# hkust-vgd/scanobjectnn

Measured on NVIDIA H100. Metric: point-clouds/sec (B=32, N=2048, 15-class), higher is better.
Workload: dtype f32

## Files before the change

### scanobjectnn_b200/csrc/tc_mlp.cu

```cuda
#include <float.h>
#include <stdlib.h>

#include <atomic>
#include <type_traits>

#include "common.cuh"
#include "mlp_internal.cuh"
#include "ring_gemm.cuh"
#include "tc_common.cuh"

namespace psa {

using namespace tc;

constexpr int kMaxTcLayers = 2;


struct TcArgs {
    long long groups;
    int K;
    int n, m;
    const float* xyz;
    const float* new_xyz;
    const float* uf;
// ... 674 lines not shown
                    }
                }
            } else {
#pragma unroll
                for (int e = 0; e < 2; ++e) {
                    const float m = warp_rowmax16(u.v[0] ? y[0][e] : -FLT_MAX, u.v[1] ? y[1][e] : -FLT_MAX);
                    if (g == 0) sm.red[0][warp][cl + e] = m;
                }
            }
        }
        if (a.pool_k == 1) {
            if (a.stat_partial != nullptr) {
                unit_bar_sync(1, kRingConsumers);
                if (tid < 64) {
                    const int cl = cl0 + tid;
                    float t0 = 0.f, t1 = 0.f;
                    for (int w = 0; w < 8; ++w) { t0 += sm.red[0][w][cl]; t1 += sm.red[1][w][cl]; }
                    float* dst = a.stat_partial + (size_t)u.tile * 2 * a.N;
                    dst[u.col0 + cl] = t0;
                    dst[a.N + u.col0 + cl] = t1;
                }
            }
        } else {
            unit_bar_sync(1, kRingConsumers);
            const bool big = a.pool_k > 128;
            const int wpg = big ? 8 : a.pool_k / 16;
            for (int e = tid; e < (8 / wpg) * 64; e += kRingConsumers) {
                const int grp = e / 64, cl = cl0 + e % 64;
                const long long rs = u.tile * 128 + grp * wpg * 16;
                if (rs >= a.rows) continue;
                float mx = sm.red[0][grp * wpg][cl];
                for (int w = 1; w < wpg; ++w) mx = fmaxf(mx, sm.red[0][grp * wpg + w][cl]);
                const long long wg = rs / a.pool_k;
                if (!big) {
                    a.out[(size_t)wg * a.N + u.col0 + cl] = mx;
                } else {
                    int code = __float_as_int(mx);
                    code = code >= 0 ? code : code ^ 0x7fffffff;
                    atomicMax(reinterpret_cast<int*>(a.out) + (size_t)wg * a.N + u.col0 + cl, code);
                }
            }
        }
    }
};

template <int NP, int NC>
__global__ void __launch_bounds__(kRingThreads, 1) tc_dense_kernel(const __grid_constant__ TcDenseArgs a) {
    ring_gemm<NP, NC>(DenseOp<NP, NC>{a}, a.ring);
}

static_assert(ring_stages(2, 1, DenseOp<2, 1>::kBudget) == 4 && ring_stages(3, 1, DenseOp<3, 1>::kBudget) == 3 &&
              ring_stages(2, 2, DenseOp<2, 2>::kBudget) == 3 && ring_stages(3, 2, DenseOp<3, 2>::kBudget) == 2, "stages of the dense ring");
static const RingKernels kDenseRing = {{{(const void*)tc_dense_kernel<2, 1>, (const void*)tc_dense_kernel<2, 2>},
                                        {(const void*)tc_dense_kernel<3, 1>, (const void*)tc_dense_kernel<3, 2>}},
                                       "tc_dense_kernel", DenseOp<2, 1>::kBudget};

bool tc_dense_eligible(long long rows, int K, int N, int pool_k) {
    if (rows < 128 || K < 32 || N < 64 || (N % 64) != 0) return false;
    if (N > 64 && (N % 128) != 0) return false;
    if (!(pool_k == 1 || pool_k == 32 || pool_k == 64 || (pool_k >= 128 && pool_k % 128 == 0))) return false;
    if (pool_k > 1 && rows % pool_k != 0) return false;
    return true;
}

static std::atomic<int> g_tc_np{2};
int tc_np() { return g_tc_np; }

static size_t tc_dense_image_off3(int K, int N) { return tc_image_alloc_bytes((K + 63) & ~63, N, 2); }
size_t tc_dense_image_bytes(int K, int N) { return tc_dense_image_off3(K, N) + tc_image_alloc_bytes((K + 63) & ~63, N, 3); }

static size_t tc_plan_image_bytes(int Kp, int N) { return g_tc_np == 2 ? tc_image_alloc_bytes(Kp, N, 2) + tc_image_alloc_bytes(Kp, N, 3) : tc_image_alloc_bytes(Kp, N, 3); }

int tc_dense_nt(long long rows, int N) {
    const bool wide = (N % 128) == 0 && 2 * ((rows + 127) / 128 * (N / 128)) > kNumSMs;
    return (wide ? 128 : 64) | image_flag(g_tc_np);
}

int build_image(int K, int Kp, int N, int Nt, const float* W, uint8_t* image, cudaStream_t st, const unsigned int* run_if) {
    if (Nt & kImageF16x2) {
        unsigned int* trailer = reinterpret_cast<unsigned int*>(image + tc_image_trailer_off(Kp, N, 2));
        float* colscale = reinterpret_cast<float*>(image + tc_image_colscale_off(Kp, N, 2));
        PSA_CUDA(cudaMemsetAsync(trailer, 0, 256, st));
        tc_col_scale_kernel<<<(N + 31) / 32, dim3(32, 8), 0, st>>>(K, N, W, colscale, trailer);
        int rc = check_launch("tc_col_scale_kernel");
        if (rc != PSA_OK) return rc;
        tc_prep_weights_kernel<2><<<(Kp * N + 255) / 256, 256, 0, st>>>(K, Kp, N, Nt & ~kImageFlags, W, colscale, image, run_if);
    } else {
        tc_prep_weights_kernel<3><<<(Kp * N + 255) / 256, 256, 0, st>>>(K, Kp, N, Nt & ~kImageFlags, W, nullptr, image, run_if);
    }
    return check_launch("tc_prep_weights_kernel");
}
const unsigned int* image_trailer(const uint8_t* image, int Kp, int N) {
    return reinterpret_cast<const unsigned int*>(image + tc_image_trailer_off(Kp, N, 2));
}
const float* image_colscale(const uint8_t* image, int Kp, int N) {
    return reinterpret_cast<const float*>(image + tc_image_colscale_off(Kp, N, 2));
}

constexpr int kTileCounterWords = PSA_MAX_MLP_LAYERS;

static long long tc_dense_units(long long rows, int N, int Nt) { return (rows + 127) / 128 * (N / Nt); }

int launch_tc_dense(long long rows, int K, int N, int pool_k, int relu, const float* x, const float* W, const float* scale,
                    const float* shift, float* out, const uint8_t* prebuilt, uint8_t* ws_img, unsigned int* flag, unsigned int* counters,
                    cudaStream_t st, const float* xyz3 = nullptr, const float* w3 = nullptr, const float* group_add = nullptr,
                    long long group_rows = 0) {
    const int Kp = (K + 63) & ~63;
    const int Nt = tc_dense_nt(rows, N) & ~kImageFlags;
    TcDenseArgs a;
    a.rows = rows; a.K = K; a.Kp = Kp; a.N = N; a.pool_k = pool_k; a.relu = relu;
    a.x = x; a.scale = scale; a.shift = shift; a.out = out; a.xyz3 = xyz3; a.w3 = w3;
    a.group_add = group_add; a.group_rows = group_rows;
    RingPool pool;
    if (pool_k > 128) { pool.out = out; pool.count = rows / pool_k * N; }
    return ring_run(kDenseRing, a, tc_dense_units(rows, N, Nt), RingWeights{K, Kp, N, Nt, W, ws_img, ws_img + tc_dense_image_off3(K, N), prebuilt},
                    flag, counters, st, pool);
}

bool tc_train_fwd_eligible(long long rows, int K, int N) {
    return rows >= 128 && K >= 128 && K <= 512 && N >= 128 && (N % 128) == 0;
}
int launch_tc_dense_train(long long rows, int K, int N, const float* x, const float* in_scale, const float* in_shift, int in_relu,
                          const float* W, const float* bias, float* y, float* stat_partial, uint8_t* image_ws, cudaStream_t st) {
    const int Kp = (K + 63) & ~63;
    int rc = build_image(K, Kp, N, 128 | kImageBf16x3, W, image_ws, st);
    if (rc != PSA_OK) return rc;
    TcDenseArgs a;
    a.rows = rows; a.K = K; a.Kp = Kp; a.N = N; a.pool_k = 1; a.relu = 0;
    a.x = x; a.scale = nullptr; a.shift = bias; a.out = y; a.xyz3 = nullptr; a.w3 = nullptr;
    a.in_scale = in_scale; a.in_shift = in_shift; a.in_relu = in_relu; a.stat_partial = stat_partial;
    a.ring.image = image_ws;
    return ring_launch(kDenseRing, 3, 128, &a, tc_dense_units(rows, N, 128), st);
}

static const uint8_t* prebuilt_image(const psa_mlp* mlp, int l, int row0, int Nt) {
    if (mlp->image[l] != nullptr && mlp->image_nt[l] == Nt && mlp->image_row0[l] == row0) return reinterpret_cast<const uint8_t*>(mlp->image[l]);
    return nullptr;
}

bool tc_sa_eligible(const psa_mlp* mlp, int c, int nsample, TcArgs* out, int np) {
    if (mlp->n_layers < 2 || mlp->n_layers > 1 + kMaxTcLayers) return false;
    if (!(nsample == 32 || nsample == 64 || nsample == 128)) return false;
    if (mlp->channels[0] != 3 + c) return false;
    const int C1 = mlp->channels[1];
    if (!(C1 == 64 || C1 == 128)) return false;
    TcArgs a{};
    a.C1 = C1;
    a.nl = mlp->n_layers - 1;
    a.np = np;
    for (int l = 0; l < a.nl; ++l) {
        a.Kd[l] = mlp->channels[1 + l];
        a.Ntot[l] = mlp->channels[2 + l];
        if (!(a.Kd[l] == 64 || a.Kd[l] == 128)) return false;
        const bool is_last = (l == a.nl - 1);
        if (!is_last && !(a.Ntot[l] == 64 || a.Ntot[l] == 128)) return false;
        if (is_last && !(a.Ntot[l] == 64 || a.Ntot[l] % 128 == 0)) return false;
    }
    a.stream_last = 0;
    if (tc_sa_layout(a).total + 1024 > kSmemBudget) a.stream_last = 1;
    if (tc_sa_layout(a).total + 1024 > kSmemBudget) return false;
    *out = a;
    return true;
}
bool tc_sa_eligible(const psa_mlp* mlp, int c, int nsample, TcArgs* out) {
    TcArgs a3;
    if (!tc_sa_eligible(mlp, c, nsample, &a3, 3)) return false;
    if (g_tc_np == 3) { *out = a3; return true; }
    return tc_sa_eligible(mlp, c, nsample, out, 2);
}

size_t tc_sa_workspace_bytes(const TcArgs& a, int b, int n, int c) {
    size_t bytes = 256;
    for (int l = 0; l < a.nl; ++l) bytes += tc_image_alloc_bytes(a.Kd[l], a.Ntot[l], 2) + tc_image_alloc_bytes(a.Kd[l], a.Ntot[l], 3);
    if (c > 0) bytes += (((size_t)b * n * a.C1 * sizeof(float) + 255) & ~(size_t)255) + tc_dense_image_bytes(c, a.C1);
    return bytes;
}

static int tc_sa_image_nt() { return kSaNt | image_flag(g_tc_np); }

template <int NP, int C1, int NL, int N0>
static int launch_tc_sa_shape(const TcArgs& a, long long ctas_needed, size_t smem, cudaStream_t st) {
    PSA_CUDA(cudaFuncSetAttribute(tc_sa_kernel<NP, C1, NL, N0>, cudaFuncAttributeMaxDynamicSharedMemorySize, (int)smem));
    int dev = 0, sms = 0, per_sm = 0;
    PSA_CUDA(cudaGetDevice(&dev));
    PSA_CUDA(cudaDeviceGetAttribute(&sms, cudaDevAttrMultiProcessorCount, dev));
    PSA_CUDA(cudaOccupancyMaxActiveBlocksPerMultiprocessor(&per_sm, tc_sa_kernel<NP, C1, NL, N0>, kSaThreads, smem));
    const long long resident = (long long)sms * (per_sm > 0 ? per_sm : 1);
    const int ctas = (int)(ctas_needed < 1 ? 1 : ctas_needed < resident ? ctas_needed : resident);
    tc_sa_kernel<NP, C1, NL, N0><<<ctas, kSaThreads, smem, st>>>(a);
    return check_launch("tc_sa_kernel");
}

template <int NP>
static int launch_tc_sa_np(TcArgs& a, cudaStream_t st) {
    const uint32_t limit = 223u * 1024u;
    a.joint = a.K == 128 || a.stream_last;
    if (!a.joint && tc_sa_layout(a).total + 1024 + sa_carry_bytes(a) + sa_red_bytes(1) > limit) a.joint = 1;
    const size_t used = (size_t)tc_sa_layout(a).total + 1024 + sa_carry_bytes(a);
    const int ncl = a.Ntot[a.nl - 1] / 64;
    a.pool_chunks = 1;
    if (!a.stream_last)
        for (int ng = ncl; ng > 1; --ng)
            if (ncl % ng == 0 && used + sa_red_bytes(ng) <= limit) { a.pool_chunks = ng; break; }
    const int C = sa_chunk(a.K, a.joint);
    const long long nchunks = (a.groups + C - 1) / C;
    const long long ctas_needed = a.joint ? nchunks : (nchunks + 1) / 2;
    const size_t smem = used + sa_red_bytes(a.pool_chunks);
    if (a.nl == 1) return a.C1 == 64 ? launch_tc_sa_shape<NP, 64, 1, 0>(a, ctas_needed, smem, st) : launch_tc_sa_shape<NP, 128, 1, 0>(a, ctas_needed, smem, st);
    if (a.C1 == 64) return a.Ntot[0] == 64 ? launch_tc_sa_shape<NP, 64, 2, 64>(a, ctas_needed, smem, st) : launch_tc_sa_shape<NP, 64, 2, 128>(a, ctas_needed, smem, st);
    return a.Ntot[0] == 64 ? launch_tc_sa_shape<NP, 128, 2, 64>(a, ctas_needed, smem, st) : launch_tc_sa_shape<NP, 128, 2, 128>(a, ctas_needed, smem, st);
}

static int tc_sa_run(TcArgs& a, int b, int n, int m, int c, int nsample, const float* xyz, const float* new_xyz, const float* points,
                     const int* idx, const psa_mlp* mlp, const float* w1c, float* out, void* workspace, cudaStream_t st) {
    int rc = PSA_OK;
    uint8_t* ws = reinterpret_cast<uint8_t*>(workspace);
    unsigned int* words = reinterpret_cast<unsigned int*>(ws);
    PSA_CUDA(cudaMemsetAsync(ws, 0, 256, st));
    ws += 256;
    uint8_t* img2[kMaxTcLayers];
    uint8_t* img3[kMaxTcLayers];
    for (int l = 0; l < a.nl; ++l) {
        img2[l] = ws; ws += tc_image_alloc_bytes(a.Kd[l], a.Ntot[l], 2);
        img3[l] = ws; ws += tc_image_alloc_bytes(a.Kd[l], a.Ntot[l], 3);
    }
    const float* uf = nullptr;
    if (c > 0) {
        float* ufw = reinterpret_cast<float*>(ws);
        uint8_t* uimg = ws + (((size_t)b * n * a.C1 * sizeof(float) + 255) & ~(size_t)255);
        const float* w1f = mlp->weight[0] + (size_t)3 * a.C1;
        if (tc_dense_eligible((long long)b * n, c, a.C1, 1)) {
            rc = launch_tc_dense((long long)b * n, c, a.C1, 1, 0, points, w1f, nullptr, nullptr, ufw, prebuilt_image(mlp, 0, 3, tc_dense_nt((long long)b * n, a.C1)),
                                 uimg, words + 3, words + 4, st);
        } else {
            DenseArgs d;
            d.rows = (long long)b * n; d.K = c; d.N = a.C1; d.pool_k = 1; d.relu = 0;
            d.x = points; d.W = w1f; d.scale = nullptr; d.shift = nullptr; d.out = ufw;
            rc = launch_dense(d, st);
        }
        if (rc != PSA_OK) return rc;
        uf = ufw;
    }
    auto fill = [&](TcArgs& t) {
        t.groups = (long long)b * m; t.K = nsample; t.n = n; t.m = m;
        t.xyz = xyz; t.new_xyz = new_xyz; t.idx = idx; t.out = out; t.uf = uf;
        t.w1x = mlp->weight[0]; t.s1 = mlp->scale[0]; t.t1 = mlp->shift[0]; t.relu1 = mlp->relu[0];
        t.ovf = nullptr; t.run_if = nullptr; t.w1c = w1c;
        for (int l = 0; l < t.nl; ++l) {
            t.s[l] = mlp->scale[1 + l]; t.t[l] = mlp->shift[1 + l]; t.relu[l] = mlp->relu[1 + l]; t.wflag[l] = nullptr; t.colscale[l] = nullptr;
        }
    };
    fill(a);
    for (int l = 0; l < a.nl; ++l) {
        const int nt_img = tc_sa_image_nt();
        const uint8_t* pre = prebuilt_image(mlp, 1 + l, 0, nt_img);
        uint8_t* own = a.np == 2 ? img2[l] : img3[l];
        if (pre == nullptr) { rc = build_image(a.Kd[l], a.Kd[l], a.Ntot[l], nt_img, mlp->weight[1 + l], own, st); if (rc != PSA_OK) return rc; }
        a.image[l] = pre ? pre : own;
        if (a.np == 2) { a.wflag[l] = image_trailer(a.image[l], a.Kd[l], a.Ntot[l]); a.colscale[l] = image_colscale(a.image[l], a.Kd[l], a.Ntot[l]); }
    }
    a.tile_counter = words;
    if (a.np == 3) return launch_tc_sa_np<3>(a, st);
    a.ovf = words + 2;
    rc = launch_tc_sa_np<2>(a, st);
    if (rc != PSA_OK) return rc;
    TcArgs a3;
    PSA_REQUIRE(tc_sa_eligible(mlp, c, nsample, &a3, 3), "sa_module: internal error (bf16x3 eligibility)");
    fill(a3);
    for (int l = 0; l < a3.nl; ++l) {
        const uint8_t* pre = prebuilt_image(mlp, 1 + l, 0, kSaNt | kImageF16x2);
        if (pre != nullptr) {
            a3.image[l] = pre + tc_image_alloc_bytes(a3.Kd[l], a3.Ntot[l], 2);
        } else {
            rc = build_image(a3.Kd[l], a3.Kd[l], a3.Ntot[l], kSaNt | kImageBf16x3, mlp->weight[1 + l], img3[l], st, words + 2);
            if (rc != PSA_OK) return rc;
            a3.image[l] = img3[l];
        }
    }
    a3.tile_counter = words + 1;
    a3.run_if = words + 2;
    return launch_tc_sa_np<3>(a3, st);
}

struct TcGroupAllArgs {
    int c;
    int N[3];
    int Nt[3];
    const float* points;
    const float* xyz;
    const float* w3;
    const uint8_t* image[3];
    const float* colscale[3];
    const unsigned int* wflag[3];
    const float* scale[3];
    const float* shift[3];
    int relu[3];
    float* out;
    unsigned int* ovf;
};

constexpr int kGaStages = 3;
constexpr uint32_t kGaStageBytes = 32768u;
constexpr uint32_t kGaSmemBudget = 222u * 1024u;
__host__ __device__ inline uint32_t group_all_smem(int W0, int W1, int W2) {
    return 1024u + kGaStages * kGaStageBytes + (uint32_t)(W0 + W1) / 64u * kRingXBytes + 12u * (uint32_t)(W0 + W1 + W2);
}

__device__ __forceinline__ uint32_t cluster_ctarank() {
    uint32_t r;
    asm volatile("mov.u32 %0, %%cluster_ctarank;\n" : "=r"(r));
    return r;
}
__device__ __forceinline__ uint32_t mapa_shared(uint32_t addr, uint32_t rank) {
    uint32_t r;
    asm volatile("mapa.shared::cluster.u32 %0, %1, %2;\n" : "=r"(r) : "r"(addr), "r"(rank));
    return r;
}
__device__ __forceinline__ float2 ld_cluster_f32x2(uint32_t addr) {
    float2 v;
    asm volatile("ld.shared::cluster.v2.f32 {%0, %1}, [%2];\n" : "=f"(v.x), "=f"(v.y) : "r"(addr) : "memory");
    return v;
}
__device__ __forceinline__ void cluster_sync_all() {
    asm volatile("barrier.cluster.arrive.release.aligned;\n\tbarrier.cluster.wait.acquire.aligned;\n" ::: "memory");
}
__device__ __forceinline__ void mbar_arrive_cluster(uint32_t addr) {
    asm volatile("fence.acq_rel.cluster;\n\tmbarrier.arrive.release.cluster.shared::cluster.b64 _, [%0];\n" ::"r"(addr) : "memory");
}
__device__ __forceinline__ void mbar_wait_cluster(uint64_t* bar, uint32_t parity) {
    uint32_t done;
    const uint32_t addr = smem_u32(bar);
    do {
        asm volatile(
            "{\n\t.reg .pred p;\n\t"
            "mbarrier.try_wait.parity.acquire.cluster.shared::cta.b64 p, [%1], %2;\n\t"
            "selp.u32 %0, 1, 0, p;\n\t}\n"
            : "=r"(done)
            : "r"(addr), "r"(parity)
            : "memory");
    } while (!done);
}

template <int NC0, int NC1>
__global__ void __cluster_dims__(4, 1, 1) __launch_bounds__(kRingThreads, 1)
tc_group_all_kernel(const __grid_constant__ TcGroupAllArgs a) {
    constexpr int NP = 2, S = kGaStages;
    constexpr uint32_t piece = 8192u, chunk = 16384u;
    extern __shared__ uint8_t smem_raw[];
    __shared__ __align__(8) uint64_t s_full[S], s_empty[S], s_ready[2], s_done;
    __shared__ float s_red[8][128];
    const int tid = threadIdx.x, lane = tid & 31, warp = tid >> 5;
    const uint32_t rank = cluster_ctarank();
    const int cloud = blockIdx.x >> 2;
    uint8_t* base = smem_raw + ((1024u - (smem_u32(smem_raw) & 1023u)) & 1023u);
    constexpr int W0 = 64 * NC0, W1 = 64 * NC1;
    const int W2 = a.N[2] / 4;
    uint8_t* slice0 = base + S * kGaStageBytes;
    uint8_t* slice1 = slice0 + NC0 * kRingXBytes;
    float* aff0 = reinterpret_cast<float*>(slice1 + NC1 * kRingXBytes);
    float* aff1 = aff0 + 3 * W0;
    float* aff2 = aff1 + 3 * W1;
    {
        float* aff[3] = {aff0, aff1, aff2};
        const int W[3] = {W0, W1, W2};
#pragma unroll
        for (int l = 0; l < 3; ++l)
            for (int i = tid; i < W[l]; i += kRingThreads) {
                const int col = (int)rank * W[l] + i;
                const float cs = __ldg(a.colscale[l] + col);
                aff[l][i] = (a.scale[l] ? __ldg(a.scale[l] + col) : 1.f) * cs;
                aff[l][W[l] + i] = a.shift[l] ? __ldg(a.shift[l] + col) : 0.f;
                aff[l][2 * W[l] + i] = pow2_rcp(cs);
            }
    }
    if (tid == 0) {
        for (int i = 0; i < S; ++i) { mbar_init(&s_full[i], 1); mbar_init(&s_empty[i], kRingConsumers / 32); }
        mbar_init(&s_ready[0], 4); mbar_init(&s_ready[1], 4); mbar_init(&s_done, 4);
        fence_mbar_init();
    }
    __syncthreads();
    cluster_sync_all();
    const int KC[3] = {a.c / 64, 4 * W0 / 64, 4 * W1 / 64};

    if (warp >= kRingConsumers / 32) {
        asm volatile("setmaxnreg.dec.sync.aligned.u32 40;\n");
        if (warp != kRingConsumers / 32) return;
        uint32_t u = 0;
#pragma unroll
        for (int l = 0; l < 3; ++l) {
            const int pw = l == 0 ? W0 : l == 1 ? W1 : 128, passes = l == 2 ? W2 / 128 : 1, Nt = a.Nt[l];
            for (int p = 0; p < passes; ++p) {
                const int j0 = ((int)rank * (l == 0 ? W0 : l == 1 ? W1 : W2) + p * pw) / 64;
                for (int kb = 0; kb < KC[l]; ++kb, ++u) {
                    const int s = (int)(u % S);
                    if (u >= (uint32_t)S) mbar_wait(&s_empty[s], ((u / S) - 1u) & 1u);
                    if (lane == 0) {
                        mbar_expect_tx(&s_full[s], (uint32_t)(pw / 64) * chunk);
                        for (int c = 0; c < pw / 64; ++c) {
                            uint8_t* dst = base + (uint32_t)s * kGaStageBytes + (uint32_t)c * chunk;
                            const int j = j0 + c;
                            if (Nt == 64) {
                                bulk_g2s(dst, a.image[l] + ((size_t)j * KC[l] + kb) * chunk, chunk, &s_full[s]);
                            } else {
                                const uint8_t* src = a.image[l] + ((size_t)(j >> 1) * KC[l] + kb) * (2u * chunk) + (uint32_t)(j & 1) * piece;
                                bulk_g2s(dst, src, piece, &s_full[s]);
                                bulk_g2s(dst + piece, src + 2u * piece, piece, &s_full[s]);
                            }
                        }
                    }
                }
            }
        }
        return;
    }

    asm volatile("setmaxnreg.inc.sync.aligned.u32 232;\n");
    const int g = lane >> 2, t = lane & 3;
    const int rl[2] = {warp * 16 + g, warp * 16 + g + 8};
    uint32_t ovf = 0u;
    uint32_t u = 0;

    auto pass = [&](auto Ltag, auto NCtag, int lc) {
        constexpr int L = decltype(Ltag)::value, NC = decltype(NCtag)::value;
        const int nkb = KC[L];
        auto prep = [&](uint32_t (&A)[NP][4][4], int kb) {
            if constexpr (L == 0) {
                const float* xb = a.points + (size_t)cloud * 128 * a.c + kb * 64;
#pragma unroll
                for (int s = 0; s < 4; ++s)
#pragma unroll
                    for (int h = 0; h < 2; ++h)
#pragma unroll
                        for (int i = 0; i < 2; ++i) {
                            const float2 x = __ldg(reinterpret_cast<const float2*>(xb + (size_t)rl[i] * a.c + 16 * s + 8 * h + 2 * t));
                            put_a<NP, 4>(A, s, i + 2 * h, x.x, x.y, ovf);
                        }
            } else {
                constexpr int Wp = L == 1 ? W0 : W1;
                const uint32_t src = mapa_shared(smem_u32(L == 1 ? slice0 : slice1) + (uint32_t)((kb * 64) % Wp / 64) * kRingXBytes,
                                                 (uint32_t)(kb * 64 / Wp));
#pragma unroll
                for (int s = 0; s < 4; ++s)
#pragma unroll
                    for (int h = 0; h < 2; ++h)
#pragma unroll
                        for (int i = 0; i < 2; ++i) {
                            const float2 x = ld_cluster_f32x2(src + (uint32_t)rl[i] * kRingXRow + (uint32_t)(16 * s + 8 * h + 2 * t) * 4u);
                            put_a<NP, 4>(A, s, i + 2 * h, x.x, x.y, ovf);
                        }
            }
        };
        float acc[NC][32];
        auto step = [&](const uint32_t (&A)[NP][4][4], uint32_t (&An)[NP][4][4], int kb) {
            const int s = (int)(u % S);
            mbar_wait(&s_full[s], (u / S) & 1u);
            const uint32_t wb = smem_u32(base) + (uint32_t)s * kGaStageBytes;
            float d[NC][32];
            wg_fence();
#pragma unroll
            for (int tt = 0; tt < Split<NP>::kTerms; ++tt)
#pragma unroll
                for (int ks = 0; ks < 4; ++ks)
#pragma unroll
                    for (int c = 0; c < NC; ++c)
                        wg_mma_rs<NP>(d[c], A[Split<NP>::a(tt)][ks][0], A[Split<NP>::a(tt)][ks][1], A[Split<NP>::a(tt)][ks][2], A[Split<NP>::a(tt)][ks][3],
                                      wg_desc(wb + (uint32_t)c * chunk + Split<NP>::w(tt) * piece + (uint32_t)ks * 32u), (tt | ks) ? 1u : 0u);
            wg_commit();
            if (kb + 1 < nkb) prep(An, kb + 1);
            wg_wait_all();
            __syncwarp();
            if (lane == 0) mbar_arrive1(&s_empty[s]);
            ++u;
#pragma unroll
            for (int c = 0; c < NC; ++c) {
                wg_fence_acc(d[c]);
#pragma unroll
                for (int e = 0; e < 32; ++e) acc[c][e] = kb ? acc[c][e] + d[c][e] : d[c][e];
            }
        };
        {
            uint32_t A0[NP][4][4], A1[NP][4][4];
            prep(A0, 0);
            for (int kb = 0;; kb += 2) {
                step(A0, A1, kb);
                if (kb + 1 == nkb) break;
                step(A1, A0, kb + 1);
                if (kb + 2 == nkb) break;
            }
        }

        constexpr int W = L == 0 ? W0 : L == 1 ? W1 : 0;
        const int Wl = L == 2 ? W2 : W;
        const float* aff = L == 0 ? aff0 : L == 1 ? aff1 : aff2;
        float xs[2][3] = {{0.f, 0.f, 0.f}, {0.f, 0.f, 0.f}};
        if constexpr (L == 0)
#pragma unroll
            for (int i = 0; i < 2; ++i)
#pragma unroll
                for (int k = 0; k < 3; ++k) xs[i][k] = __ldg(a.xyz + ((size_t)cloud * 128 + rl[i]) * 3 + k);
#pragma unroll
        for (int c = 0; c < NC; ++c)
#pragma unroll
            for (int j = 0; j < 8; ++j) {
                const int cl = c * 64 + 8 * j + 2 * t, ls = lc + cl;
                float y[2][2];
#pragma unroll
                for (int e = 0; e < 2; ++e) {
                    const float sc = aff[ls + e], sh = aff[Wl + ls + e];
                    float w0 = 0.f, w1 = 0.f, w2 = 0.f;
                    if constexpr (L == 0) {
                        const int col = (int)rank * W0 + ls + e;
                        const float f = aff[2 * Wl + ls + e];
                        w0 = __ldg(a.w3 + col) * f; w1 = __ldg(a.w3 + a.N[0] + col) * f; w2 = __ldg(a.w3 + 2 * a.N[0] + col) * f;
                    }
#pragma unroll
                    for (int i = 0; i < 2; ++i) {
                        float x = acc[c][4 * j + 2 * i + e];
                        if constexpr (L == 0) x = fmaf(xs[i][2], w2, fmaf(xs[i][1], w1, fmaf(xs[i][0], w0, x)));
                        x = fmaf(x, sc, sh);
                        if (a.relu[L]) x = fmaxf(x, 0.f);
                        y[i][e] = x;
                    }
                }
                if constexpr (L < 2) {
                    uint8_t* sl = (L == 0 ? slice0 : slice1) + (ls >> 6) * kRingXBytes + (ls & 63) * 4;
#pragma unroll
                    for (int i = 0; i < 2; ++i) *reinterpret_cast<float2*>(sl + rl[i] * kRingXRow) = make_float2(y[i][0], y[i][1]);
                } else {
#pragma unroll
                    for (int e = 0; e < 2; ++e) {
                        const float m = warp_rowmax16(y[0][e], y[1][e]);
                        if (g == 0) s_red[warp][cl + e] = m;
                    }
                }
            }
        unit_bar_sync(1, kRingConsumers);
        if constexpr (L < 2) {
            if (tid < 4) mbar_arrive_cluster(mapa_shared(smem_u32(&s_ready[L]), (uint32_t)tid));
            mbar_wait_cluster(&s_ready[L], 0);
        } else {
            for (int cl = tid; cl < 64 * NC; cl += kRingConsumers) {
                float mx = s_red[0][cl];
                for (int w = 1; w < 8; ++w) mx = fmaxf(mx, s_red[w][cl]);
                a.out[(size_t)cloud * a.N[2] + (size_t)rank * W2 + lc + cl] = mx;
            }
            unit_bar_sync(1, kRingConsumers);
        }
    };
    pass(std::integral_constant<int, 0>{}, std::integral_constant<int, NC0>{}, 0);
    pass(std::integral_constant<int, 1>{}, std::integral_constant<int, NC1>{}, 0);
    for (int lc = 0; lc < W2; lc += 128) pass(std::integral_constant<int, 2>{}, std::integral_constant<int, 2>{}, lc);

    if (tid < 4) mbar_arrive_cluster(mapa_shared(smem_u32(&s_done), (uint32_t)tid));
    if (f16x2_overflowed(ovf) || (tid == 0 && (*a.wflag[0] | *a.wflag[1] | *a.wflag[2]) != 0u)) atomicOr(a.ovf, 1u);
    mbar_wait_cluster(&s_done, 0);
}

template <int NC0, int NC1>
static size_t group_all_fits(const psa_mlp* mlp) {
    const size_t smem = group_all_smem(64 * NC0, 64 * NC1, mlp->channels[3] / 4);
    if (smem > kGaSmemBudget) return 0;
    if (cudaFuncSetAttribute(tc_group_all_kernel<NC0, NC1>, cudaFuncAttributeMaxDynamicSharedMemorySize, (int)smem) != cudaSuccess) return 0;
    cudaLaunchConfig_t cfg = {};
    cfg.gridDim = dim3(4, 1, 1);
    cfg.blockDim = dim3(kRingThreads, 1, 1);
    cfg.dynamicSmemBytes = smem;
    int clusters = 0;
    if (cudaOccupancyMaxActiveClusters(&clusters, tc_group_all_kernel<NC0, NC1>, &cfg) != cudaSuccess) { (void)cudaGetLastError(); return 0; }
    return clusters > 0 ? smem : 0;
}
static size_t group_all_eligible(int n, int c, const float* points, const psa_mlp* mlp) {
    if (g_tc_np != 2 || mlp->n_layers != 3 || n != 128 || c < 64 || c % 64 != 0 || (reinterpret_cast<uintptr_t>(points) & 15) != 0) return 0;
    const int N0 = mlp->channels[1], N1 = mlp->channels[2], N2 = mlp->channels[3];
    if (N2 % 512 != 0) return 0;
    if (N0 == 256 && N1 == 256) return group_all_fits<1, 1>(mlp);
    if (N0 == 256 && N1 == 512) return group_all_fits<1, 2>(mlp);
    if (N0 == 512 && N1 == 256) return group_all_fits<2, 1>(mlp);
    return 0;
}

static int sa_group_all_cluster(int b, int c, const float* xyz, const float* points, const psa_mlp* mlp, float* out, float* ws0, float* ws1,
                                uint8_t* img, unsigned int* words, size_t smem, cudaStream_t st) {
    const long long rows = (long long)b * 128;
    unsigned int* flag = words + kTileCounterWords - 1;
    TcGroupAllArgs g{};
    g.c = c; g.points = points; g.xyz = xyz; g.w3 = mlp->weight[0]; g.out = out; g.ovf = flag;
    const uint8_t* pre[3];
    uint8_t* ws_img[3];
    int rc;
    for (int l = 0; l < 3; ++l) {
        const int K = l == 0 ? c : mlp->channels[l], N = mlp->channels[l + 1], Nt = tc_dense_nt(rows, N);
        const float* W = l == 0 ? mlp->weight[0] + (size_t)3 * N : mlp->weight[l];
        pre[l] = prebuilt_image(mlp, l, l == 0 ? 3 : 0, Nt);
        ws_img[l] = img;
        img += tc_dense_image_bytes(K, N);
        if (pre[l] == nullptr) { rc = build_image(K, K, N, Nt, W, ws_img[l], st); if (rc != PSA_OK) return rc; }
        const uint8_t* image = pre[l] ? pre[l] : ws_img[l];
        g.N[l] = N; g.Nt[l] = Nt & ~kImageFlags; g.image[l] = image;
        g.colscale[l] = image_colscale(image, K, N); g.wflag[l] = image_trailer(image, K, N);
        g.scale[l] = mlp->scale[l]; g.shift[l] = mlp->shift[l]; g.relu[l] = mlp->relu[l];
    }
    const int N0 = mlp->channels[1], N1 = mlp->channels[2];
    if (N0 == 256 && N1 == 256) tc_group_all_kernel<1, 1><<<4u * (unsigned)b, kRingThreads, smem, st>>>(g);
    else if (N0 == 256) tc_group_all_kernel<1, 2><<<4u * (unsigned)b, kRingThreads, smem, st>>>(g);
    else tc_group_all_kernel<2, 1><<<4u * (unsigned)b, kRingThreads, smem, st>>>(g);
    rc = check_launch("tc_group_all_kernel");
    if (rc != PSA_OK) return rc;
    const float* cur = points;
    for (int l = 0; l < 3; ++l) {
        const int K = l == 0 ? c : mlp->channels[l], N = mlp->channels[l + 1];
        TcDenseArgs a;
        a.rows = rows; a.K = K; a.Kp = K; a.N = N; a.pool_k = l == 2 ? 128 : 1; a.relu = mlp->relu[l];
        a.x = cur; a.scale = mlp->scale[l]; a.shift = mlp->shift[l]; a.out = l == 2 ? out : (l & 1) ? ws1 : ws0;
        a.xyz3 = l == 0 ? xyz : nullptr; a.w3 = l == 0 ? mlp->weight[0] : nullptr;
        const RingWeights w{K, K, N, g.Nt[l], l == 0 ? mlp->weight[0] + (size_t)3 * N : mlp->weight[l], ws_img[l],
                            ws_img[l] + tc_dense_image_off3(K, N), pre[l]};
        rc = ring_rerun(kDenseRing, a, tc_dense_units(rows, N, g.Nt[l]), w, flag, words + kTileCounterWords + 2 * l + 1, st);
        if (rc != PSA_OK) return rc;
        cur = a.out;
    }
    return PSA_OK;
}

}

using namespace psa;

static std::atomic<int> g_mlp_mode{0};
int psa::mlp_mode() { return g_mlp_mode; }
extern "C" PSA_API int psa_set_mlp_mode(int mode) {
    PSA_REQUIRE(mode == 0 || mode == 1 || mode == 2,
                "set_mlp_mode: mode must be 0 (tensor cores, fp16x2 operands with the range guard), 1 (fp32 FMA kernels only) or 2 (tensor cores, bf16x3)");
    g_mlp_mode = mode;
    g_tc_np = mode == 2 ? 3 : 2;
    return PSA_OK;
}
extern "C" PSA_API int psa_get_mlp_mode(void) { return g_mlp_mode; }

extern "C" size_t psa_sa_module_workspace_bytes(int b, int n, int m, int c, int nsample, const psa_mlp* mlp) {
    (void)m;
    TcArgs a;
    if (g_mlp_mode != 1 && mlp != nullptr && tc_sa_eligible(mlp, c, nsample, &a)) return tc_sa_workspace_bytes(a, b, n, c);
    return 0;
}

extern "C" int psa_sa_module_infer(int b, int n, int m, int c, float radius, int nsample, const float* xyz,
                                   const float* new_xyz, const float* points, const int* idx_in, const psa_mlp* mlp,
                                   float* out, int* idx_out, int* pts_cnt, void* workspace, size_t workspace_bytes,
                                   psa_stream_t stream) {
    int rc = validate_mlp_public(mlp, "sa_module");
    if (rc != PSA_OK) return rc;
    PSA_REQUIRE(b >= 0 && n >= 1 && m >= 0 && c >= 0 && nsample >= 1, "sa_module: bad dims b=%d n=%d m=%d c=%d nsample=%d", b, n, m, c, nsample);
    PSA_REQUIRE(mlp->channels[0] == 3 + c, "sa_module: mlp input width %d != 3 + c (%d)", mlp->channels[0], 3 + c);
    if (b == 0 || m == 0) return PSA_OK;
    PSA_REQUIRE(xyz && new_xyz && out && (points || c == 0), "sa_module: null buffer");
    const int* idx = idx_in;
    if (idx == nullptr) {
        PSA_REQUIRE(idx_out != nullptr, "sa_module: idx_out must be provided when idx_in is NULL (it receives the ball query)");
        rc = psa_query_ball_point(b, n, m, radius, nsample, xyz, new_xyz, idx_out, pts_cnt, stream);
        if (rc != PSA_OK) return rc;
        idx = idx_out;
    }
    cudaStream_t st = as_stream(stream);
    TcArgs a;
    if (g_mlp_mode != 1 && tc_sa_eligible(mlp, c, nsample, &a)) {
        const size_t need = tc_sa_workspace_bytes(a, b, n, c);
        PSA_REQUIRE(workspace != nullptr && workspace_bytes >= need,
                    "sa_module: workspace of %zu bytes required (psa_sa_module_workspace_bytes), got %zu", need, workspace_bytes);
        PSA_REQUIRE((reinterpret_cast<uintptr_t>(workspace) & 255) == 0, "sa_module: workspace must be 256-byte aligned");
        return tc_sa_run(a, b, n, m, c, nsample, xyz, new_xyz, points, idx, mlp, nullptr, out, workspace, st);
    }
    return sa_module_simt(b, n, m, c, nsample, xyz, new_xyz, points, idx, mlp, out, st);
}

extern "C" size_t psa_shared_mlp_workspace_bytes(long long rows, const psa_mlp* mlp) {
    if (mlp == nullptr || mlp->n_layers < 1) return 0;
    size_t bytes = 0;
    int cmax = 0;
    for (int l = 1; l < mlp->n_layers; ++l) cmax = cmax > mlp->channels[l] ? cmax : mlp->channels[l];
    if (mlp->n_layers > 1) bytes += 2 * (((size_t)rows * cmax * sizeof(float) + 255) & ~(size_t)255);
    for (int l = 0; l < mlp->n_layers; ++l) bytes += tc_dense_image_bytes(mlp->channels[l], mlp->channels[l + 1] < 64 ? 64 : mlp->channels[l + 1]);
    if (rows <= 32) {
        size_t fc = 0;
        for (int l = 0; l < mlp->n_layers; ++l) { size_t f = fc_small_workspace_bytes(mlp->channels[l], mlp->channels[l + 1]); fc = f > fc ? f : fc; }
        bytes += (fc + 255) & ~(size_t)255;
    }
    return bytes + 256;
}

static int shared_mlp_chain(long long rows, int pool_k, const float* x, const psa_mlp* mlp, const float* group_add, long long group_rows,
                            float* out, void* workspace, size_t workspace_bytes, psa_stream_t stream) {
    int rc;
    const int L = mlp->n_layers;
    const size_t need = psa_shared_mlp_workspace_bytes(rows, mlp);
    PSA_REQUIRE(workspace != nullptr && workspace_bytes >= need, "shared_mlp: workspace of %zu bytes required (got %zu)", need, workspace_bytes);
    PSA_REQUIRE((reinterpret_cast<uintptr_t>(workspace) & 255) == 0, "shared_mlp: workspace must be 256-byte aligned");
    int cmax = 0;
    for (int l = 1; l < L; ++l) cmax = cmax > mlp->channels[l] ? cmax : mlp->channels[l];
    const size_t half = L > 1 ? (((size_t)rows * cmax * sizeof(float) + 255) & ~(size_t)255) : 0;
    uint8_t* wsb = reinterpret_cast<uint8_t*>(workspace);
    float* ws0 = reinterpret_cast<float*>(wsb);
    float* ws1 = reinterpret_cast<float*>(wsb + half);
    uint8_t* img = wsb + 2 * half;
    float* fc_partial = nullptr;
    if (rows <= 32) {
        size_t imgs = 0;
        for (int l = 0; l < L; ++l) imgs += tc_dense_image_bytes(mlp->channels[l], mlp->channels[l + 1] < 64 ? 64 : mlp->channels[l + 1]);
        fc_partial = reinterpret_cast<float*>(img + imgs);
    }
    const float* cur = x;
    cudaStream_t st = as_stream(stream);
    unsigned int* flags = reinterpret_cast<unsigned int*>(wsb + need - 256);
    PSA_CUDA(cudaMemsetAsync(flags, 0, 256, st));
    for (int l = 0; l < L; ++l) {
        const int K = mlp->channels[l], N = mlp->channels[l + 1];
        const int pk = (l == L - 1) ? pool_k : 1;
        float* dst = (l == L - 1) ? out : ((l & 1) ? ws1 : ws0);
        const float* gadd = l == 0 ? group_add : nullptr;
        if (g_mlp_mode != 1 && tc_dense_eligible(rows, K, N, pk)) {
            rc = launch_tc_dense(rows, K, N, pk, mlp->relu[l], cur, mlp->weight[l], mlp->scale[l], mlp->shift[l], dst, prebuilt_image(mlp, l, 0, tc_dense_nt(rows, N)),
                                 img, flags + l, flags + kTileCounterWords + 2 * l, st, nullptr, nullptr, gadd, group_rows);
        } else {
            DenseArgs d;
            d.rows = rows; d.K = K; d.N = N; d.pool_k = pk; d.relu = mlp->relu[l];
            d.x = cur; d.W = mlp->weight[l]; d.scale = mlp->scale[l]; d.shift = mlp->shift[l]; d.out = dst;
            d.group_add = gadd; d.group_rows = group_rows;
            rc = (rows <= 32 && pk == 1 && gadd == nullptr) ? launch_fc_small(d, fc_partial, st) : launch_dense(d, st);
        }
        if (rc != PSA_OK) return rc;
        img += tc_dense_image_bytes(K, N < 64 ? 64 : N);
        cur = dst;
    }
    return PSA_OK;
}

extern "C" int psa_shared_mlp(long long rows, int pool_k, const float* x, const psa_mlp* mlp, float* out,
                              void* workspace, size_t workspace_bytes, psa_stream_t stream) {
    int rc = validate_mlp_public(mlp, "shared_mlp");
    if (rc != PSA_OK) return rc;
    PSA_REQUIRE(rows >= 0 && pool_k >= 1, "shared_mlp: rows=%lld pool_k=%d", rows, pool_k);
    if (rows == 0) return PSA_OK;
    PSA_REQUIRE(rows % pool_k == 0, "shared_mlp: rows=%lld is not a multiple of pool_k=%d", rows, pool_k);
    PSA_REQUIRE(x && out, "shared_mlp: null buffer");
    return shared_mlp_chain(rows, pool_k, x, mlp, nullptr, 0, out, workspace, workspace_bytes, stream);
}

extern "C" int psa_shared_mlp_grouped(long long rows, long long group_rows, const float* x, const psa_mlp* mlp, const float* group_add,
                                      float* out, void* workspace, size_t workspace_bytes, psa_stream_t stream) {
    int rc = validate_mlp_public(mlp, "shared_mlp_grouped");
    if (rc != PSA_OK) return rc;
    PSA_REQUIRE(rows >= 0 && group_rows >= 1, "shared_mlp_grouped: rows=%lld group_rows=%lld", rows, group_rows);
    PSA_REQUIRE(rows % group_rows == 0, "shared_mlp_grouped: group_rows=%lld does not divide rows=%lld", group_rows, rows);
    if (rows == 0) return PSA_OK;
    PSA_REQUIRE(x && group_add && out, "shared_mlp_grouped: null buffer");
    return shared_mlp_chain(rows, 1, x, mlp, group_add, group_rows, out, workspace, workspace_bytes, stream);
}

extern "C" size_t psa_sa_group_all_workspace_bytes(int b, int n, int c, const psa_mlp* mlp) {
    if (mlp == nullptr || mlp->n_layers < 1) return 0;
    psa_mlp m2 = *mlp;
    m2.channels[0] = c;
    return psa_shared_mlp_workspace_bytes((long long)b * n, &m2);
}

extern "C" int psa_sa_group_all_infer(int b, int n, int c, const float* xyz, const float* points, const psa_mlp* mlp,
                                      float* out, void* workspace, size_t workspace_bytes, psa_stream_t stream) {
    int rc = validate_mlp_public(mlp, "sa_group_all");
    if (rc != PSA_OK) return rc;
    PSA_REQUIRE(b >= 0 && n >= 1 && c >= 1, "sa_group_all: bad dims b=%d n=%d c=%d", b, n, c);
    PSA_REQUIRE(mlp->channels[0] == 3 + c, "sa_group_all: mlp input width %d != 3 + c (%d)", mlp->channels[0], 3 + c);
    if (b == 0) return PSA_OK;
    PSA_REQUIRE(xyz && points && out, "sa_group_all: null buffer");
    const long long rows = (long long)b * n;
    const int L = mlp->n_layers;
    const int N0 = mlp->channels[1];
    const int pk0 = (L == 1) ? n : 1;
    PSA_SUPPORTED(g_mlp_mode != 1 && tc_dense_eligible(rows, c, N0, pk0),
                  "sa_group_all: first layer (%d -> %d over %lld rows) is not eligible for the tensor-core path; concatenate and use shared_mlp", c, N0, rows);
    const size_t need = psa_sa_group_all_workspace_bytes(b, n, c, mlp);
    PSA_REQUIRE(workspace != nullptr && workspace_bytes >= need, "sa_group_all: workspace of %zu bytes required (got %zu)", need, workspace_bytes);
    PSA_REQUIRE((reinterpret_cast<uintptr_t>(workspace) & 255) == 0, "sa_group_all: workspace must be 256-byte aligned");
    int cmax = 0;
    for (int l = 1; l < L; ++l) cmax = cmax > mlp->channels[l] ? cmax : mlp->channels[l];
    const size_t half = L > 1 ? (((size_t)rows * cmax * sizeof(float) + 255) & ~(size_t)255) : 0;
    uint8_t* wsb = reinterpret_cast<uint8_t*>(workspace);
    float* ws0 = reinterpret_cast<float*>(wsb);
    float* ws1 = reinterpret_cast<float*>(wsb + half);
    uint8_t* img = wsb + 2 * half;
    cudaStream_t st = as_stream(stream);
    unsigned int* flags = reinterpret_cast<unsigned int*>(wsb + need - 256);
    PSA_CUDA(cudaMemsetAsync(flags, 0, 256, st));
    if (g_mlp_mode == 0) {
        const size_t smem = group_all_eligible(n, c, points, mlp);
        if (smem != 0) return sa_group_all_cluster(b, c, xyz, points, mlp, out, ws0, ws1, img, flags, smem, st);
    }
    const float* cur = points;
    for (int l = 0; l < L; ++l) {
        const int K = (l == 0) ? c : mlp->channels[l], N = mlp->channels[l + 1];
        const int pk = (l == L - 1) ? n : 1;
        float* dst = (l == L - 1) ? out : ((l & 1) ? ws1 : ws0);
        const float* W = (l == 0) ? mlp->weight[0] + (size_t)3 * N : mlp->weight[l];
        if (tc_dense_eligible(rows, K, N, pk)) {
            rc = launch_tc_dense(rows, K, N, pk, mlp->relu[l], cur, W, mlp->scale[l], mlp->shift[l], dst, prebuilt_image(mlp, l, l == 0 ? 3 : 0, tc_dense_nt(rows, N)),
                                 img, flags + l, flags + kTileCounterWords + 2 * l, st, l == 0 ? xyz : nullptr, l == 0 ? mlp->weight[0] : nullptr);
        } else {
            PSA_SUPPORTED(l > 0, "sa_group_all: layer 0 must run on the tensor-core path");
            DenseArgs d;
            d.rows = rows; d.K = K; d.N = N; d.pool_k = pk; d.relu = mlp->relu[l];
            d.x = cur; d.W = W; d.scale = mlp->scale[l]; d.shift = mlp->shift[l]; d.out = dst;
            rc = launch_dense(d, st);
        }
        if (rc != PSA_OK) return rc;
        img += tc_dense_image_bytes(K, N < 64 ? 64 : N);
        cur = dst;
    }
    return PSA_OK;
}

__global__ void edge_wc_kernel(int c, int N, const float* __restrict__ W, float* __restrict__ Wc) {
    const int total = c * 2 * N;
    for (int e = blockIdx.x * blockDim.x + threadIdx.x; e < total; e += gridDim.x * blockDim.x) {
        const int kk = e / (2 * N), j = e - kk * 2 * N;
        Wc[e] = j < N ? __ldg(W + (size_t)kk * N + j) - __ldg(W + (size_t)(c + kk) * N + j) : __ldg(W + (size_t)(c + kk) * N + j - N);
    }
}

template <int VEC>
__global__ void __launch_bounds__(256)
edge_gather_max_kernel(long long points, int n, int k, int N, const float* __restrict__ AB, const int* __restrict__ nn_idx,
                       const float* __restrict__ scale, const float* __restrict__ shift, int relu, float* __restrict__ out) {
    const int lane = threadIdx.x & 31;
    const long long warp0 = (long long)blockIdx.x * 8 + (threadIdx.x >> 5);
    float sc[VEC], sh[VEC];
#pragma unroll
    for (int v = 0; v < VEC; ++v) {
        sc[v] = scale ? __ldg(scale + lane * VEC + v) : 1.f;
        sh[v] = shift ? __ldg(shift + lane * VEC + v) : 0.f;
    }
// ... 147 lines not shown
```

Before: 92960.

## Store group-all layer activations as pre-split MMA fragments in shared memory

Intermediate activations of the group-all MLP are now written in the epilogue already split into the NP-term register-fragment layout, stored with 16-byte vector stores per warp and lane. The next layer's A-operand prep then loads whole fragments with v4 loads, using plain shared loads when the slice is local and cluster DSMEM loads otherwise. This removes the per-element float2 DSMEM loads and the split/convert work in the MMA prep, which sits on the critical path between wgmma issue and wait. In exchange, each slice's shared-memory footprint changes to a fixed 32KB, and optional clock64 timestamp instrumentation is compiled in only under a macro.

Result: faster. 97070, median of 6 (+4.4%).

```diff
diff --git a/scanobjectnn_b200/csrc/tc_mlp.cu b/scanobjectnn_b200/csrc/tc_mlp.cu
--- a/scanobjectnn_b200/csrc/tc_mlp.cu
+++ b/scanobjectnn_b200/csrc/tc_mlp.cu
@@ -1000,8 +1000,10 @@
 constexpr int kGaStages = 3;
 constexpr uint32_t kGaStageBytes = 32768u;
 constexpr uint32_t kGaSmemBudget = 222u * 1024u;
+constexpr uint32_t kGaSliceBytes = 32768u;
+__device__ __forceinline__ uint32_t ga_frag_off(int warp, int lane, int q) { return (uint32_t)(((warp * 8 + q) * 32 + lane) * 16); }
 __host__ __device__ inline uint32_t group_all_smem(int W0, int W1, int W2) {
-    return 1024u + kGaStages * kGaStageBytes + (uint32_t)(W0 + W1) / 64u * kRingXBytes + 12u * (uint32_t)(W0 + W1 + W2);
+    return 1024u + kGaStages * kGaStageBytes + (uint32_t)(W0 + W1) / 64u * kGaSliceBytes + 12u * (uint32_t)(W0 + W1 + W2);
 }
 
 __device__ __forceinline__ uint32_t cluster_ctarank() {
@@ -1014,10 +1016,14 @@
     asm volatile("mapa.shared::cluster.u32 %0, %1, %2;\n" : "=r"(r) : "r"(addr), "r"(rank));
     return r;
 }
-__device__ __forceinline__ float2 ld_cluster_f32x2(uint32_t addr) {
-    float2 v;
-    asm volatile("ld.shared::cluster.v2.f32 {%0, %1}, [%2];\n" : "=f"(v.x), "=f"(v.y) : "r"(addr) : "memory");
-    return v;
+__device__ __forceinline__ void ld_cluster_v4(uint32_t addr, uint32_t (&v)[4]) {
+    asm volatile("ld.shared::cluster.v4.u32 {%0, %1, %2, %3}, [%4];\n" : "=r"(v[0]), "=r"(v[1]), "=r"(v[2]), "=r"(v[3]) : "r"(addr) : "memory");
+}
+__device__ __forceinline__ void ld_shared_v4(uint32_t addr, uint32_t (&v)[4]) {
+    asm volatile("ld.shared.v4.u32 {%0, %1, %2, %3}, [%4];\n" : "=r"(v[0]), "=r"(v[1]), "=r"(v[2]), "=r"(v[3]) : "r"(addr) : "memory");
+}
+__device__ __forceinline__ void st_shared_v4(uint32_t addr, const uint32_t (&v)[4]) {
+    asm volatile("st.shared.v4.u32 [%0], {%1, %2, %3, %4};\n" ::"r"(addr), "r"(v[0]), "r"(v[1]), "r"(v[2]), "r"(v[3]) : "memory");
 }
 __device__ __forceinline__ void cluster_sync_all() {
     asm volatile("barrier.cluster.arrive.release.aligned;\n\tbarrier.cluster.wait.acquire.aligned;\n" ::: "memory");
@@ -1038,6 +1044,34 @@
             : "memory");
     } while (!done);
 }
+
+#ifdef PSA_GA_STAMPS
+constexpr int kGaStampCtas = 256, kGaStampUses = 64;
+__device__ long long g_ga_stamps[kGaStampCtas][2][kGaStampUses][4];
+extern "C" PSA_API int psa_group_all_stamps(long long* dst) {
+    return cudaMemcpyFromSymbol(dst, g_ga_stamps, sizeof(g_ga_stamps)) == cudaSuccess ? 0 : 1;
+}
+#define GA_STAMP(u, k)                                                                                              \
+    do {                                                                                                            \
+        if ((threadIdx.x & 127) == 0 && blockIdx.x < kGaStampCtas && (u) < kGaStampUses)                            \
+            g_ga_stamps[blockIdx.x][threadIdx.x >> 7][(u)][(k)] = clock64();                                        \
+    } while (0)
+#define GA_STAMP_AFTER(u, k, r)                                                                                     \
+    do {                                                                                                            \
+        if ((threadIdx.x & 127) == 0 && blockIdx.x < kGaStampCtas && (u) < kGaStampUses) {                          \
+            volatile long long* p_ = &g_ga_stamps[blockIdx.x][threadIdx.x >> 7][(u)][(k)];                          \
+            *p_ = (long long)__float_as_uint(__fmul_rn(__uint_as_float(r), 0.f));                                   \
+            *p_ = clock64();                                                                                        \
+        }                                                                                                           \
+    } while (0)
+#else
+#define GA_STAMP(u, k) \
+    do {               \
+    } while (0)
+#define GA_STAMP_AFTER(u, k, r) \
+    do {                        \
+    } while (0)
+#endif
 
 template <int NC0, int NC1>
 __global__ void __cluster_dims__(4, 1, 1) __launch_bounds__(kRingThreads, 1)
@@ -1054,8 +1088,8 @@
     constexpr int W0 = 64 * NC0, W1 = 64 * NC1;
     const int W2 = a.N[2] / 4;
     uint8_t* slice0 = base + S * kGaStageBytes;
-    uint8_t* slice1 = slice0 + NC0 * kRingXBytes;
-    float* aff0 = reinterpret_cast<float*>(slice1 + NC1 * kRingXBytes);
+    uint8_t* slice1 = slice0 + NC0 * kGaSliceBytes;
+    float* aff0 = reinterpret_cast<float*>(slice1 + NC1 * kGaSliceBytes);
     float* aff1 = aff0 + 3 * W0;
     float* aff2 = aff1 + 3 * W1;
     {
@@ -1117,6 +1151,7 @@
     const int rl[2] = {warp * 16 + g, warp * 16 + g + 8};
     uint32_t ovf = 0u;
     uint32_t u = 0;
+    GA_STAMP(kGaStampUses - 1, 0);
 
     auto pass = [&](auto Ltag, auto NCtag, int lc) {
         constexpr int L = decltype(Ltag)::value, NC = decltype(NCtag)::value;
@@ -1135,23 +1170,23 @@
                         }
             } else {
                 constexpr int Wp = L == 1 ? W0 : W1;
-                const uint32_t src = mapa_shared(smem_u32(L == 1 ? slice0 : slice1) + (uint32_t)((kb * 64) % Wp / 64) * kRingXBytes,
-                                                 (uint32_t)(kb * 64 / Wp));
-#pragma unroll
-                for (int s = 0; s < 4; ++s)
-#pragma unroll
-                    for (int h = 0; h < 2; ++h)
-#pragma unroll
-                        for (int i = 0; i < 2; ++i) {
-                            const float2 x = ld_cluster_f32x2(src + (uint32_t)rl[i] * kRingXRow + (uint32_t)(16 * s + 8 * h + 2 * t) * 4u);
-                            put_a<NP, 4>(A, s, i + 2 * h, x.x, x.y, ovf);
-                        }
+                const uint32_t owner = (uint32_t)(kb * 64 / Wp);
+                const uint32_t src = smem_u32(L == 1 ? slice0 : slice1) + (uint32_t)((kb * 64) % Wp / 64) * kGaSliceBytes + ga_frag_off(warp, lane, 0);
+                if (owner == rank) {
+#pragma unroll
+                    for (int q = 0; q < NP * 4; ++q) ld_shared_v4(src + (uint32_t)q * 512u, A[q >> 2][q & 3]);
+                } else {
+                    const uint32_t rsrc = mapa_shared(src, owner);
+#pragma unroll
+                    for (int q = 0; q < NP * 4; ++q) ld_cluster_v4(rsrc + (uint32_t)q * 512u, A[q >> 2][q & 3]);
+                }
             }
         };
         float acc[NC][32];
         auto step = [&](const uint32_t (&A)[NP][4][4], uint32_t (&An)[NP][4][4], int kb) {
             const int s = (int)(u % S);
             mbar_wait(&s_full[s], (u / S) & 1u);
+            GA_STAMP(u, 0);
             const uint32_t wb = smem_u32(base) + (uint32_t)s * kGaStageBytes;
             float d[NC][32];
             wg_fence();
@@ -1164,8 +1199,11 @@
                         wg_mma_rs<NP>(d[c], A[Split<NP>::a(tt)][ks][0], A[Split<NP>::a(tt)][ks][1], A[Split<NP>::a(tt)][ks][2], A[Split<NP>::a(tt)][ks][3],
                                       wg_desc(wb + (uint32_t)c * chunk + Split<NP>::w(tt) * piece + (uint32_t)ks * 32u), (tt | ks) ? 1u : 0u);
             wg_commit();
+            GA_STAMP(u, 1);
             if (kb + 1 < nkb) prep(An, kb + 1);
+            GA_STAMP_AFTER(u, 2, An[1][3][3]);
             wg_wait_all();
+            GA_STAMP(u, 3);
             __syncwarp();
             if (lane == 0) mbar_arrive1(&s_empty[s]);
             ++u;
@@ -1197,7 +1235,8 @@
 #pragma unroll
                 for (int k = 0; k < 3; ++k) xs[i][k] = __ldg(a.xyz + ((size_t)cloud * 128 + rl[i]) * 3 + k);
 #pragma unroll
-        for (int c = 0; c < NC; ++c)
+        for (int c = 0; c < NC; ++c) {
+            uint32_t fr[NP][4];
 #pragma unroll
             for (int j = 0; j < 8; ++j) {
                 const int cl = c * 64 + 8 * j + 2 * t, ls = lc + cl;
@@ -1221,9 +1260,18 @@
                     }
                 }
                 if constexpr (L < 2) {
-                    uint8_t* sl = (L == 0 ? slice0 : slice1) + (ls >> 6) * kRingXBytes + (ls & 63) * 4;
-#pragma unroll
-                    for (int i = 0; i < 2; ++i) *reinterpret_cast<float2*>(sl + rl[i] * kRingXRow) = make_float2(y[i][0], y[i][1]);
+#pragma unroll
+                    for (int i = 0; i < 2; ++i) {
+                        uint32_t p[NP];
+                        split_pair<NP>(y[i][0], y[i][1], p, ovf);
+#pragma unroll
+                        for (int pc = 0; pc < NP; ++pc) fr[pc][i + 2 * (j & 1)] = p[pc];
+                    }
+                    if (j & 1) {
+                        const uint32_t sl = smem_u32(L == 0 ? slice0 : slice1) + (uint32_t)c * kGaSliceBytes;
+#pragma unroll
+                        for (int pc = 0; pc < NP; ++pc) st_shared_v4(sl + ga_frag_off(warp, lane, 4 * pc + (j >> 1)), fr[pc]);
+                    }
                 } else {
 #pragma unroll
                     for (int e = 0; e < 2; ++e) {
@@ -1232,6 +1280,7 @@
                     }
                 }
             }
+        }
         unit_bar_sync(1, kRingConsumers);
         if constexpr (L < 2) {
             if (tid < 4) mbar_arrive_cluster(mapa_shared(smem_u32(&s_ready[L]), (uint32_t)tid));
```
